# engyasin/EKF-MonoSLAM_for_3D-reconstruction

Measured on AMD Instinct MI355X. Metric: EKF updates/sec at N features (state dim 14+6N), higher is better.
Workload: dtype f32 (state, covariance, every accumulation and every other contraction in fp32; the products of the covariance downdate as 3 x bf16 splits of the fp32 operands, six bf16 products per fp32 product: the dropped terms are <= 2^-24 |a||b| in the worst case (2^-28 on average) -- the size of the fp32 prod; 1 GPU; N=1000 inverse-depth features, n=6014, M=N measured per frame, fp32, 1xMI355X (BASELINE configs[2]); features=1000, state_dim=6014, measured_per_frame=1000, camera=conf_kinect.cfg/scale2, frames_per_map=3000, maps=1

## Files before the change

### ekf-monoslam_for_3d-reconstruction_amd/csrc/ekf_capi.hip

```cpp
#include <hip/hip_runtime.h>

#include <algorithm>
#include <array>
#include <climits>
#include <cmath>
#include <cstdint>
#include <cstdio>
#include <cstdlib>
#include <cstring>
#include <map>
#include <mutex>
#include <string>
#include <type_traits>
#include <vector>

#include "../../include/ekf_monoslam.h"
#include "ekf_buffers.hpp"
#include "ekf_feature_table.hpp"
#include "ekf_dense.hpp"
#include "ekf_image.hpp"
#include "ekf_features.hpp"
#include "ekf_syrk6.hpp"
#include "ekf_chain.hpp"
#include "ekf_small.hpp"
// ... 41 lines not shown
  KID_SEED_MASK,
  KID_SEED_RESPONSE,
  KID_SEED_CANDIDATES,
  KID_SEED_SELECT,
  KID_FRAME_UPLOAD,
  KID_FRAME_INGEST,
  KID_FRAME_RECTIFY,
  KID_COUNT
};

static const char* kKernelNames[KID_COUNT] = {
    "predict_camera",  "propagate_strips", "propagate_streaming", "measure",
    "innovation",      "sigma_ht",         "innovation_cov",      "chol_diag",
    "chol_panel",      "chol_trailing",    "state_update",        "downdate_syrk",
    "solve_trmm",      "normalize_quat",  "add_feature",      "compact_transform",   "misc",
    "w_update", "allgather_h", "allgather_s", "allgather_v", "allgather_sigma",
    "seed_mask", "seed_response", "seed_candidates", "seed_select", "frame_upload", "frame_ingest", "frame_rectify"};

static const char* kLaunchNames[EKF_LAUNCH_KINDS] = {
    "downdate_bf16x6", "downdate_f32", "downdate_f32_fused_wu", "downdate_f32_half_tail", "downdate_f32_t64",
    "row_rider", "row_gemv", "row_tile_gemm", "w_update_gemm", "w_recompute",
    "chain_step_launches", "chain_persistent", "solve", "solve_two_groups", "update_oneblock", "update_allinone",
    "chain_trail_diag", "split_image", "state_update_tail", "update_onelaunch", "chain_dist_gather", "chain_step_fused",
    "downdate_mirror_bounds", "solve_poll_chain"};

static inline int round_up(int v, int a) { return (v + a - 1) / a * a; }

struct MaskedStreamPool {
  struct Entry { int device, num_cus, reserved; hipStream_t st; };
  std::mutex mu;
  std::vector<Entry> idle;
  bool hooked = false;
  static void at_exit();
  hipStream_t take(int device, int num_cus, int reserved) {
    std::lock_guard<std::mutex> lk(mu);
    for (size_t i = 0; i < idle.size(); ++i)
      if (idle[i].device == device && idle[i].num_cus == num_cus && idle[i].reserved == reserved) {
        hipStream_t st = idle[i].st;
        idle.erase(idle.begin() + i);
        return st;
      }
    return nullptr;
  }
  void give(int device, int num_cus, int reserved, hipStream_t st) {
    std::lock_guard<std::mutex> lk(mu);
    idle.push_back({device, num_cus, reserved, st});
    if (!hooked) { hooked = true; atexit(&MaskedStreamPool::at_exit); }
// ... 170 lines not shown
  DevBuf<unsigned char> d_raw;
  int raw_w = 0, raw_h = 0, raw_c = 0;
  bool have_raw = false;
  RectScratch rect;
  DevBuf<int4> d_ingest_tab;
  int ingest_tab_w = 0, ingest_tab_h = 0;
  DevBuf<unsigned char> d_patch[2], d_mpatch[2];
  int cur_patch = 0;
  DevBuf<T> d_hb, d_zm;
  DevBuf<unsigned char> d_found;
  DevBuf<float> d_score;
  DevBuf<int> d_keep;
  int opt_panel_direct = 1;
  int opt_chain_fused_diag = 1;
  int opt_small_onelaunch = 1;
  int opt_step_fused = 1;
  struct StepPlan { std::vector<int> off, cnt; } sfp;
  WorkList sf_lists{{0}, {}};
  DevBuf<unsigned long long> d_small_stamps;
  unsigned small_gate_total = 0;
  int opt_su_tail = 1;
  int opt_syrk_mirror_skip = 1;
  int opt_solve_poll_chain = 1;
  int opt_fuse_split = 1;
  int opt_chain_defer = 1;
  int td_min_blocks = 24;
  int td_max_blocks = 1 << 30;
  WorkList td_blocks;
  std::vector<int> td_off, td_cnt;
  int opt_syrk_stag_half = 0, opt_syrk_stag_mod4 = 2;
  int opt_solve_s2 = 1;
  bool want_solve_s2(int width, int npad_live) const {
    return kIsF32 && opt_mfma && opt_solve_s2 && (opt_solve_s2 > 1 || (width / 128) * (npad_live / 64) <= 2 * num_cus);
  }
  int opt_fused = 1;
  int opt_solve_one_per_cu = 1;
  int opt_wrecompute = 1;
  int opt_row_gemv = 1;
  int opt_fuse_wu = 1;
  int env_chunks[8] = {}, env_nchunks = 0;
  int opt_pipeline = -1;
  WorkList tilemap{{0, 0}, {}};
  int tri_count = 0, solve_off = 0;
  int w_zeroed_n = -1;
  DevBuf<int> d_counters;
  int num_cus = 256, reserved_cus = 32;
// ... 125 lines not shown
          stream_b = nullptr;
          reserved_cus = 0;
          HIPCHK(hipStreamCreateWithFlags(&stream_b, hipStreamNonBlocking));
        }
      }
      stream_b_reserved = reserved_cus;

      if (const char* e = getenv("EKF_FUSE_WU")) opt_fuse_wu = atoi(e);
      if (const char* e = getenv("EKF_ROW_GEMV")) opt_row_gemv = atoi(e) ? 1 : 0;
      if (const char* e = getenv("EKF_SOLVE_ONE_PER_CU")) opt_solve_one_per_cu = atoi(e) ? 1 : 0;
      if (const char* e = getenv("EKF_W_RECOMPUTE")) opt_wrecompute = atoi(e) ? 1 : 0;
      if (const char* e = getenv("EKF_SOLVE_S2")) opt_solve_s2 = atoi(e);
      if (const char* e = getenv("EKF_FUSED_LAUNCHES")) opt_fused = atoi(e) ? 1 : 0;
      if (const char* e = getenv("EKF_PANEL_DIRECT")) opt_panel_direct = atoi(e);
      if (const char* e = getenv("EKF_SYRK_STAGGER")) {
        opt_syrk_stag_half = atoi(e);
        if (const char* c = strchr(e, ',')) opt_syrk_stag_mod4 = atoi(c + 1);
      }
      if (const char* e = getenv("EKF_CHAIN_FUSED_DIAG")) opt_chain_fused_diag = atoi(e) ? 1 : 0;
      if (const char* e = getenv("EKF_FUSE_SPLIT")) opt_fuse_split = atoi(e) ? 1 : 0;
      if (const char* e = getenv("EKF_SU_TAIL")) opt_su_tail = atoi(e) ? 1 : 0;
      if (const char* e = getenv("EKF_SYRK_MIRROR_SKIP")) opt_syrk_mirror_skip = atoi(e) ? 1 : 0;
      if (const char* e = getenv("EKF_SOLVE_POLL_CHAIN")) opt_solve_poll_chain = std::max(0, std::min(2, atoi(e)));
      if (const char* e = getenv("EKF_SMALL_ONELAUNCH")) opt_small_onelaunch = atoi(e) ? 1 : 0;
      if (const char* e = getenv("EKF_STEP_FUSED")) opt_step_fused = atoi(e) ? 1 : 0;
      if (const char* e = getenv("EKF_SHARD_DIST_CHAIN")) opt_shard_dist_chain = atoi(e) ? 1 : 0;
      if (const char* e = getenv("EKF_SHARD_DIST_MIN_BLOCKS")) shard_dist_min_blocks = std::max(2, atoi(e));
      if (const char* e = getenv("EKF_SMALL_STAMPS")) {
        if (atoi(e)) { HIPCHK(d_small_stamps.reserve(16)); HIPCHK(hipMemset(d_small_stamps, 0, 16 * sizeof(unsigned long long))); }
      }
      if (const char* e = getenv("EKF_CHAIN_DEFER")) opt_chain_defer = atoi(e) ? 1 : 0;
      if (const char* e = getenv("EKF_TD_MIN_BLOCKS")) td_min_blocks = std::max(1, atoi(e));
      if (const char* e = getenv("EKF_TD_MAX_BLOCKS")) td_max_blocks = std::max(1, atoi(e));
      if (const char* e = getenv("EKF_SPLIT_TAIL")) opt_split_tail = atoi(e);
      if (const char* e = getenv("EKF_SPLIT_BF16")) opt_split_bf16 = atoi(e) ? 1 : 0;
      if (const char* e = getenv("EKF_CHUNKS")) {
        for (const char* q = e; *q && env_nchunks < 8;) {
          env_chunks[env_nchunks++] = atoi(q);
          while (*q && *q != ',') ++q;
          if (*q == ',') ++q;
        }
      }
    }
    std::vector<T> mu0(camera_dim, T(0));
    mu0[3] = T(0.0); mu0[4] = T(0.0); mu0[5] = T(-0.707106781); mu0[6] = T(0.707106781);
    if (camera_dim == 14) mu0[13] = T(1);
// ... 683 lines not shown
      int rc = zero_border(dst, n);
      if (rc) return rc;
      cur = dst;
    } else {
      Scope sc(this, KID_PROPAGATE_STRIPS);
      k_strip_congruence<T, 13><<<(2 * n + 255) / 256, 256, 0, stream>>>(S(), ld, n, 0, d_scr + SCR_FT, d_scr + SCR_Q);
    }
    if (opt_feature_noise > 0.0 && n > camera_dim)
      k_inflate_diagonal<T><<<(n - camera_dim + 255) / 256, 256, 0, stream>>>(S(), ld, camera_dim, n, T(opt_feature_noise));
    HIPCHK(hipGetLastError());
    return EKF_OK;
  }

  int predict(const void* tc, const void* rc_, int vcontrol) override {
    HIPCHK(hipSetDevice(device));
    if (sh_on) return shard_predict(tc, rc_, vcontrol);
    const MotionArgs a = motion_args(tc, rc_, vcontrol);
    if (opt_fused && !opt_streaming && !(opt_feature_noise > 0.0) && N > 0 && !prof.on(KID_PREDICT_CAMERA) &&
        !prof.on(KID_PROPAGATE_STRIPS) && !prof.on(KID_MEASURE)) {
      int rc = sync_layout();
      if (rc) return rc;
      const int nstrip = (2 * n + 255) / 256;
      k_predict_fused<T><<<nstrip + (N + 255) / 256, 256, 0, stream>>>(mu(), d_scr, a, S(), ld, n, nstrip, d_pos, d_coding, N,
                                                                      cam, d_h, d_Hc, d_Hf, d_flags, d_status + 8, d_status);
      HIPCHK(hipGetLastError());
      rc = launch_track_fold();
      if (rc) return rc;
      have_motion = true;
      have_update = false;
      have_meas = true;
      have_sd = false;
      return launch_blur();
    }
    int rcp = propagate(a, opt_streaming);
    if (rcp) return rcp;
    have_update = false;
    int rcm = launch_measure();
    if (rcm) return rcm;
    return launch_blur();
  }

  int measure() override {
    HIPCHK(hipSetDevice(device));
    return launch_measure();
  }

  bool have_motion = false;
  int motion_jacobian(void* Ft, void* Q) override {
    HIPCHK(hipSetDevice(device));
    if (!have_motion) FAIL(EKF_ERR_STATE, "no motion Jacobian: call ekf_predict first");
// ... 84 lines not shown
    int nb = 0, tile = 0, m = 0, m_pad = 0, npad_live = 0, nsteps = 0;
    int nchunks = 1, cend[8] = {};
    ChunkTab tab{};
    int strip_rows = 0;
    int ntr = 0, ntc = 0;
    bool oneblock = false, allinone = false, onelaunch = false;
    int small_rc = 0, small_nchunk = 0, small_nt64 = 0;
    bool recompute = false;
    int r0 = 0, r1 = 0, p0 = 0, prows = 0;
    Rows ranges[3] = {};
    bool sym_panel = false, shard_split = false;
    int c0(int g) const { return (g ? cend[g - 1] : 0) * nb; }
    int c1(int g) const { return cend[g] * nb; }
  };
  struct UpdateCtx {
    const T* z;
    const int* midx;
    int* counters;
    int counter_next = 0;
    bool step_fused = false;
    int diag_ahead = -1;
    struct { int step = -1, c0 = 0, c1 = 0; } pending;
    bool row_pending = false;
    bool queue_room(int ints = 8) const { return counter_next + ints <= kQueueCounters; }
    int* take_queue() {
      if (!queue_room()) return nullptr;
      counter_next += 8;
      return counters + counter_next - 8;
    }
  };

  template <int ROLE, bool BT, int TM = 128, int TN = 128>
  void gemm(const GemmCall& c) {
    GemmArgs g{};
    g.A = c.A; g.lda = c.lda; g.B = c.B; g.ldb = c.ldb; g.C = c.C; g.ldc = c.ldc;
    g.K = c.K; g.alpha = double(c.alpha); g.beta = double(c.beta);
    g.tri = c.tri; g.row_off = c.row_off; g.col_off = c.col_off; g.ktri = c.ktri; g.ktile_off = c.ktile_off;
    g.zrow = c.zrow; g.zcol_end = c.zcol_end;
    g.stagger = (ROLE == ROLE_DOWNDATE) ? 1 : 0;
    g.img = c.img; g.img_nkc = c.img_nkc; g.img_c0 = c.img_c0;
    g.chain_word = c.chain_word; g.chain_epoch = c.chain_epoch; g.status = d_status;
    hipStream_t st = c.st ? c.st : stream;
    const bool mf = kIsF32 && opt_mfma;
    dim3 grid(c.cols / (mf ? TN : 64), c.rows / (mf ? TM : 64));
    if (c.tile_list && c.counter) {
      g.tile_map = c.tile_list;
// ... 6 lines not shown
    }
    if constexpr (kIsF32) {
      if (opt_mfma) {
        if constexpr (ROLE == ROLE_SOLVE) {
          ++launch_cnt[c.two_groups ? EKF_LAUNCH_SOLVE_TWO_GROUPS : EKF_LAUNCH_SOLVE];
          if (c.two_groups) {
            k_gemm_mfma<ROLE, BT, TM, TN, true><<<grid, 512, 0, st>>>(g);
            return;
          }
        }
        k_gemm_mfma<ROLE, BT, TM, TN><<<grid, 256, 0, st>>>(g);
        return;
      }
    }
    if constexpr (!kIsF32) {
      if (opt_mfma) {
        k_gemm_mfma_f64<ROLE, BT><<<grid, 256, 0, st>>>(g);
        return;
      }
    }
    k_gemm_valu<T, ROLE, BT><<<grid, 256, 0, st>>>(g);
  }

  void launch_panel(T* P, const T* Dj, int vrows, hipStream_t st) {
    const int nb = NB();
    if constexpr (kIsF32) {
      if (opt_mfma && nb == 128 && opt_panel_direct) {
        k_panel_direct<<<(vrows + 63) / 64, 256, 0, st>>>(P, ldy, Dj, vrows);
        return;
      }
    }
    if constexpr (!kIsF32) {
      if (opt_mfma && nb == 64 && opt_panel_direct) {
        k_panel_direct_f64<<<(vrows + 63) / 64, 256, 0, st>>>(P, ldy, Dj, vrows);
        return;
      }
    }
    GemmCall c;
    c.A = P; c.lda = ldy; c.B = Dj; c.ldb = nb; c.C = P; c.ldc = ldy;
    c.rows = vrows; c.cols = nb; c.K = nb; c.st = st;
    gemm<ROLE_PANEL, false, 64, 128>(c);
  }

  int ensure_tilemap(int nt, int ntr, int ntc) {
    const std::vector<int> key = {nt, ntc};
    if (tilemap.current(key)) return EKF_OK;
    std::vector<int> tm;
    const int SB = 8;
    const int ns = (nt + SB - 1) / SB;
    for (int si = 0; si < ns; ++si)
      for (int sj = 0; sj <= si; ++sj)
// ... 279 lines not shown
      if (ux.diag_ahead != step) {
        Scope sc(this, KID_CHOL_DIAG, sc_);
        ++launch_cnt[EKF_LAUNCH_CHAIN_STEP];
        if (nb == 128) {
          if constexpr (kIsF32)
            k_chol_diag_packed<><<<1, 1024, 0, sc_>>>(Ajj, ldy, Dj, d_status, std::max(1, std::min(8, (m - j + 15) / 16)));
        } else {
          if constexpr (!kIsF32) {
            if (opt_mfma)
              k_chol_diag_packed_f64<<<1, 512, 0, sc_>>>(Ajj, ldy, Dj, d_status, std::max(1, std::min(4, (m - j + 15) / 16)));
            else
              k_chol_diag<T, 64><<<1, 512, diag_lds(64), sc_>>>(Ajj, ldy, Dj, d_status);
          } else {
            k_chol_diag<T, 64><<<1, 512, diag_lds(64), sc_>>>(Ajj, ldy, Dj, d_status);
          }
        }
      }
      const int r0 = j + nb;
      const int vrows = m_pad - c0;
      if (!skip_panel) {
        Scope sc(this, KID_CHOL_PANEL, sc_);
        T* P = Y + (size_t)r0 * ldy + j;
        ++launch_cnt[EKF_LAUNCH_CHAIN_STEP];
        launch_panel(P, Dj, vrows, sc_);
      }
      if (defer_last && step == step1 - 1 && r0 < m_pad) {
        ux.pending.step = step; ux.pending.c0 = c0; ux.pending.c1 = c1;
      } else {
        chain_trailing(ux, step, c0, c1, m, m_pad, sc_, !skip_panel);
      }
    }
  }
  int check_list(const int* idx, int M, bool ascending) {
    for (int k = 0; k < M; ++k) {
      if (idx[k] < 0 || idx[k] >= N) FAIL(EKF_ERR_ARG, "feature index out of range");
      if (ascending && k > 0 && idx[k - 1] >= idx[k]) FAIL(EKF_ERR_ARG, "measured indices must be strictly ascending");
    }
    return EKF_OK;
  }

  void launch_row_update(int c0, int c1, int m_pad, hipStream_t ss, bool gemv) {
    const size_t yrow = (size_t)round_up(n, NB()) * ldy;
    Scope sc(this, KID_WUPDATE, ss);
    ++launch_cnt[gemv ? EKF_LAUNCH_ROW_GEMV : EKF_LAUNCH_ROW_TILE_GEMM];
    if constexpr (kIsF32) {
      if (gemv) {
        k_innov_row_update<<<(m_pad - c1 + 63) / 64, 64, 0, ss>>>(d_V + yrow + c0, d_Y + (size_t)c1 * ldy + c0, ldy,
// ... 24 lines not shown
      Syrk6Args a{d_Vimg, ldy / 16, c0 / 16, width / 16, S(), ld, tiles, ntiles, head, cam_rows, r0, r1};
      a.stag_half = opt_syrk_stag_half; a.stag_mod4 = opt_syrk_stag_mod4;
      if (su_tail) {
        a.su_mu = mu(); a.su_V = d_V; a.su_ldy = ldy; a.su_n = n; a.su_y = d_V + (size_t)npad_live * ldy; a.su_mpad = m_pad;
        a.su_qn = d_scr + SCR_QN; a.su_counter = head + 1;
        ++launch_cnt[EKF_LAUNCH_STATE_UPDATE_TAIL];
      }
      if (rider) {
        a.ry = d_V + (size_t)npad_live * ldy + c0; a.rL = d_Y + (size_t)c1 * ldy + c0; a.rldl = ldy;
        a.rnu = d_W + (size_t)npad_live * ldy + c1; a.rcols = m_pad - c1; a.rK = width; a.nrider = (m_pad - c1 + 255) / 256;
        ++launch_cnt[EKF_LAUNCH_ROW_RIDER];
      }
      if (mirror_rows) {
        a.mirror_rows = mirror_rows;
        ++launch_cnt[EKF_LAUNCH_DOWNDATE_MIRROR_BOUNDS];
      }
      ++launch_cnt[EKF_LAUNCH_DOWNDATE_BF16X6];
      const int wgs = 2 * (ss == stream_b ? num_cus - reserved_cus : num_cus);
      k_syrk_bf16x6<0><<<a.nrider + std::min(ntiles, wgs), 256, 0, ss>>>(a);
    }
    return EKF_OK;
  }

  void launch_w_recompute(int c1, int c2, int m_pad, const int* list, int M, int plane, hipStream_t ss, int rows0,
                          int row0 = 0, int row1 = 0) {
    if constexpr (kIsF32) {
      Scope sc(this, KID_SIGMA_HT, ss);
      ++launch_cnt[EKF_LAUNCH_W_RECOMPUTE];
      const int s0 = c1 / 2, s1 = c2 / 2;
      const int range[2][2] = {{0, rows0}, {row0, row1}};
      for (const auto& r : range) {
        if (r[1] <= r[0]) continue;
        constexpr int RB = 8;
        dim3 grid((s1 - s0 + 127) / 128, (r[1] - r[0] + RB - 1) / RB);
        k_sigma_ht_fast<RB><<<grid, 256, 0, ss>>>(S(), ld, r[1], d_Hc, d_Hf, d_pos, d_coding, list, M, plane, d_W, ldy, m_pad, N,
                                                   s0, s1, nullptr, nullptr, nullptr, nullptr, nullptr, nullptr, nullptr, r[0]);
      }
    }
  }

  void launch_state_update(int m_pad, hipStream_t st) {
    Scope sc(this, KID_STATE_UPDATE, st);
    k_state_update<T><<<(n + 7) / 8, 512, 0, st>>>(mu(), d_V, ldy, n, d_V + (size_t)round_up(n, NB()) * ldy, m_pad, d_scr + SCR_QN);
  }

  int finish_update(const UpdatePlan& p, bool state_update, bool normalize) {
    last_nchunks = p.nchunks;
    last_recompute = p.recompute;
    for (int g = 0; g < p.nchunks; ++g) last_cend[g] = p.cend[g];
    if (state_update) launch_state_update(p.m_pad, stream);
    if (normalize) {
      Scope sc(this, KID_NORMALIZE);
      k_strip_congruence<T, 4><<<(2 * n + 255) / 256, 256, 0, stream>>>(S(), ld, n, 3, d_scr + SCR_QN,
                                                                       static_cast<const T*>(nullptr));
    }
    HIPCHK(hipGetLastError());
    last_m = p.m; last_m_pad = p.m_pad; last_n = n;
    have_update = true;
    have_meas = false;
// ... 54 lines not shown
        if (rc) return rc;
        ux.step_fused = true;
      }
    }
    return EKF_OK;
  }

  bool chunk_overlaps(const UpdatePlan& p, int g) const { return stream_b != nullptr && g + 1 < p.nchunks; }
  int chunk_slots(const UpdatePlan& p, int g) const { return 2 * (chunk_overlaps(p, g) ? num_cus - reserved_cus : num_cus); }
  bool chunk_splits(const UpdatePlan& p, const UpdateCtx& ux) const {
    return kIsF32 && opt_split_bf16 && opt_mfma && p.tile == 128 && tri_count >= num_cus && ux.queue_room();
  }
  bool chunk_fuses(const UpdatePlan& p, int g, const UpdateCtx& ux) const {
    return kIsF32 && opt_fuse_wu && (opt_fuse_wu > 1 || p.recompute || g + 2 < p.nchunks) && opt_mfma && chunk_overlaps(p, g) &&
           p.c1(g) < p.m_pad && !opt_split_bf16 && p.tile == 128 && tri_count >= num_cus && ux.queue_room();
  }
  bool chunk_row_rider(const UpdatePlan& p, int g, const UpdateCtx& ux) const {
    return chunk_splits(p, ux) && p.recompute && opt_row_gemv && p.c1(g) < p.m_pad && !chunk_fuses(p, g, ux);
  }
  bool chunk_su_tail(const UpdatePlan& p, int g, const UpdateCtx& ux) const {
    return kIsF32 && opt_su_tail && !chunk_overlaps(p, g) && p.nchunks > 1 && chunk_splits(p, ux);
  }
  bool solve_polls_chain(const UpdatePlan& p, int g) const {
    return kIsF32 && opt_mfma && opt_solve_poll_chain && (p.nsteps <= 16 || opt_solve_poll_chain > 1) && g > 0 &&
           chunk_overlaps(p, g) && stream_b_masked && reserved_cus > 0 && !p.oneblock;
  }
  enum SolveShape { SOLVE_64X64, SOLVE_128_ONE_PER_CU, SOLVE_64X128, SOLVE_128 };
  SolveShape solve_shape(const UpdatePlan& p, int g) const {
    const bool mf = kIsF32 && opt_mfma;
    const int tiles = (p.c1(g) - p.c0(g)) / p.tile * p.ntr, slots = chunk_slots(p, g);
    if (mf && 4 * tiles < slots) return SOLVE_64X64;
    if (mf && !chunk_overlaps(p, g) && opt_solve_one_per_cu && tiles < slots && tiles > num_cus) return SOLVE_128_ONE_PER_CU;
    if (mf && tiles < slots) return SOLVE_64X128;
    return SOLVE_128;
  }

  int launch_update_small(const UpdatePlan& p, const UpdateCtx& ux) {
    if constexpr (kIsF32) {
      if (w_zeroed_n != n) {
        HIPCHK(hipMemsetAsync(d_W + (size_t)n * ldy, 0, (size_t)(p.npad_live - n + p.nb) * ldy * sizeof(T), stream));
        w_zeroed_n = n;
      }
      SmallUpdateArgs a{};
      a.S = S(); a.ld = ld; a.n = n; a.npad = p.npad_live;
      a.Hc = d_Hc; a.Hf = d_Hf; a.pos = d_pos; a.coding = d_coding; a.midx = ux.midx;
      a.M = p.M; a.plane = p.plane; a.nfeat = N;
      a.z = ux.z; a.h = d_h; a.mu = mu();
      a.r_pix = T(sigma_pixel_2); a.r_plane = T(0.00001);
// ... 14 lines not shown
    const int c0 = p.c0(gi), width = p.c1(gi) - c0, ntr = p.ntr, ntc = p.ntc;
    T* Zs = d_Y + (size_t)p.m_pad * ldy;
    if (p.oneblock) {
      if constexpr (kIsF32) {
        ++launch_cnt[p.allinone ? EKF_LAUNCH_UPDATE_ALLINONE : EKF_LAUNCH_UPDATE_ONEBLOCK];
        if (p.allinone)
          k_update_oneblock_small<<<p.small_nt64 + 1, 512, 0, ss>>>(d_W, ldy, d_Dinv, d_V, ldy, p.npad_live, mu(), n, d_scr + SCR_QOLD,
                                                                   d_scr + SCR_QN, Zs, ldy, S(), ld, p.small_nt64);
        else
          k_solve_state_oneblock<<<p.npad_live / 64 + 1, 256, 0, ss>>>(d_W, ldy, d_Dinv, d_V, ldy, p.npad_live, mu(), n,
                                                                      d_scr + SCR_QN, Zs, ldy);
      }
      return EKF_OK;
    }
    Scope sc(this, KID_SOLVE, ss);
    const int wt = width / p.tile;
    GemmCall c;
    c.A = d_W + c0; c.lda = ldy; c.B = Zs + c0; c.ldb = ldy; c.C = d_V + c0; c.ldc = ldy;
    c.rows = p.npad_live + p.nb; c.cols = width; c.K = width; c.ktri = KTRI_UPPER;
    c.two_groups = want_solve_s2(width, p.npad_live);
    c.st = ss;
    if (ss == stream_b && solve_polls_chain(p, gi)) {
      c.chain_word = reinterpret_cast<const unsigned*>(d_counters + kChainEpochWord); c.chain_epoch = (unsigned)gi + 1;
      ++launch_cnt[EKF_LAUNCH_SOLVE_POLL_CHAIN];
    }
    switch (solve_shape(p, gi)) {
      case SOLVE_64X64:
        c.tile_list = tilemap.d + solve6464_off + 2 * (2 * ntc - 2 * wt) * 2 * ntr; c.ntiles = 2 * wt * 2 * ntr;
        c.counter = ux.take_queue();
        gemm<ROLE_SOLVE, true, 64, 64>(c);
        break;
      case SOLVE_128_ONE_PER_CU:
        c.tile_list = tilemap.d + solve_off + 2 * (ntc - wt) * ntr; c.ntiles = wt * ntr;
        c.counter = ux.take_queue();
        c.one_per_cu = true;
        gemm<ROLE_SOLVE, true>(c);
        break;
      case SOLVE_64X128:
        if (kIsF32 && opt_fuse_split && opt_split_bf16 && p.tile == 128 && tri_count >= num_cus && ux.queue_room(16)) {
          HIPCHK(ensure_vimg());
          c.img = d_Vimg; c.img_nkc = ldy / 16; c.img_c0 = c0;
          *vimg_done = true;
        }
        c.tile_list = tilemap.d + solve64_off + 2 * (ntc - wt) * 2 * ntr; c.ntiles = wt * 2 * ntr;
        c.counter = ux.take_queue();
        gemm<ROLE_SOLVE, true, 64, 128>(c);
        break;
// ... 104 lines not shown
    UpdateCtx ux{d_z, d_midx, d_counters};
    if (M > 0) {
      if (on_device) {
        ux.z = static_cast<const T*>(z);
        ux.midx = idx;
      } else {
        int rcs = stage_inputs(z, idx, M);
        if (rcs) return rcs;
        sh_list.clear();
      }
    }
    const UpdatePlan p = plan_update(M, plane);
    int rc = p.onelaunch ? launch_update_small(p, ux)
                         : build_innovation(ux.z, ux.midx, M, plane, true, nullptr, nullptr, &p.tab, p.strip_rows);
    if (rc) return rc;
    rc = ensure_tilemap(p.npad_live / p.tile, p.ntr, p.ntc);
    if (rc) return rc;
    rc = prepare_chain(p, ux, false);
    if (rc) return rc;
    const int nchunks = p.nchunks, m_pad = p.m_pad;
    bool b_inflight = false;
    for (int gi = 0; gi < (p.onelaunch ? 0 : nchunks); ++gi) {
      const int c0 = p.c0(gi), c1 = p.c1(gi);
      chain_steps(ux, gi ? p.cend[gi - 1] : 0, p.cend[gi], c0, c1, p.m, m_pad, stream, p.oneblock,
                  opt_chain_defer && gi + 1 < nchunks);
      const bool overlap = chunk_overlaps(p, gi);
      hipStream_t ss = overlap ? stream_b : stream;
      if (!overlap && b_inflight) {
        if (p.recompute) {
          HIPCHK(hipEventRecord(ev_b, stream_b));
          HIPCHK(hipStreamWaitEvent(stream, ev_b, 0));
          b_inflight = false;
        } else {
          HIPCHK(hipStreamWaitEvent(stream, ev_wu, 0));
        }
      }
      if (overlap) {
        b_inflight = true;
        if (solve_polls_chain(p, gi)) {
          if constexpr (kIsF32)
            k_publish_epoch<<<1, 64, 0, stream>>>(reinterpret_cast<unsigned*>(d_counters + kChainEpochWord), (unsigned)gi + 1);
        } else {
          HIPCHK(hipEventRecord(ev_chain[gi], stream));
          HIPCHK(hipStreamWaitEvent(stream_b, ev_chain[gi], 0));
        }
      }
      bool vimg_done = false;
      rc = solve_chunk(p, gi, ux, ss, &vimg_done);
      if (rc) return rc;
      const bool fuse = chunk_fuses(p, gi, ux);
      wupdate_chunk(p, gi, ux, ss);
      if (overlap && c1 < m_pad && !fuse && !p.recompute) HIPCHK(hipEventRecord(ev_wu, stream_b));
      if (!overlap && b_inflight) {
        HIPCHK(hipEventRecord(ev_b, stream_b));
        HIPCHK(hipStreamWaitEvent(stream, ev_b, 0));
        b_inflight = false;
      }
      if (!overlap && nchunks > 1 && !chunk_su_tail(p, gi, ux)) {
        HIPCHK(hipEventRecord(ev_chain[gi], stream));
        HIPCHK(hipStreamWaitEvent(stream_b, ev_chain[gi], 0));
        launch_state_update(m_pad, stream_b);
        b_inflight = true;
      }
      rc = downdate_chunk(p, gi, ux, ss, vimg_done);
// ... 3775 lines not shown
```

### ekf-monoslam_for_3d-reconstruction_amd/csrc/ekf_dense.hpp

```cpp
#pragma once
#include <type_traits>
#include "ekf_math.hpp"

namespace ekf {

typedef float f32x4 __attribute__((ext_vector_type(4)));
constexpr int kQueueCounters = 256;
constexpr int kChainEpochWord = kQueueCounters;
constexpr int kResetInts = kQueueCounters + 32;

__device__ __forceinline__ int clamp_feature(int fi, int nfeat) { return min(max(fi, 0), nfeat - 1); }
__device__ __forceinline__ void check_measured_entry(const int* __restrict__ midx, int k, int nfeat,
                                                     int* __restrict__ status) {
  const int fi = midx[k];
  if (status && (fi < 0 || fi >= nfeat || (k > 0 && midx[k - 1] >= fi))) status[1] = 1;
}

struct ChunkTab {
  int n;
  int end[8];
};

constexpr int kMirrorEmpty = 8;
constexpr int kMirrorRowsInts = 2 * (kMirrorEmpty + 1);
__device__ __forceinline__ void mirror_rows_slab(const ChunkTab& tab, const int* __restrict__ midx, int M, int nfeat,
                                                 const int* __restrict__ pos, const int* __restrict__ coding,
                                                 int* __restrict__ mrows) {
  __shared__ int s_lo[8], s_hi[8];
  const int tid = threadIdx.x;
  if (tid < 8) { s_lo[tid] = 0x7fffffff; s_hi[tid] = 0; }
  __syncthreads();
  for (int k = tid; k < M; k += blockDim.x) {
// ... 1360 lines not shown
      f4 acc = {0.f, 0.f, 0.f, 0.f};
      const float* bl = sl + (16 * ct + lr) * PITCH + 4 * lq;
#pragma unroll
      for (int u = 0; u < 8; ++u) {
        if (u <= ct) {
          const f4 fb = *reinterpret_cast<const f4*>(bl + 16 * u);
#pragma unroll
          for (int e = 0; e < 4; ++e) acc = __builtin_amdgcn_mfma_f32_16x16x4f32(fa[u][e], fb[e], acc, 0, 0, 0);
        }
      }
#pragma unroll
      for (int e = 0; e < 4; ++e) P[(size_t)(row0 + 4 * lq + e) * ldp + 16 * ct + lr] = acc[e];
    }
  };
  if (live) column_tiles(0);
#pragma unroll
  for (int p = 0; p < 8; ++p) {
    const int q = tid + 256 * p;
    *reinterpret_cast<f4*>(sl + (64 + (q >> 5)) * PITCH + 4 * (q & 31)) = v1[p];
  }
  __syncthreads();
  if (live) column_tiles(4);
}
__global__ void __launch_bounds__(256, 2) k_panel_direct(float* __restrict__ P, int ldp, const float* __restrict__ Dinv, int rows) {
  __shared__ float sl[128 * 132];
  panel_direct_body(P, ldp, Dinv, rows, blockIdx.x, sl);
}
__global__ void __launch_bounds__(256, 2) k_panel_direct_blocks(float* __restrict__ Pcol, int ldp, const float* __restrict__ Dinv,
                                                               const int* __restrict__ blocks) {
  __shared__ float sl[128 * 132];
  const int blk = blocks[blockIdx.x >> 1];
  panel_direct_body(Pcol + (size_t)blk * 128 * ldp, ldp, Dinv, 128, blockIdx.x & 1, sl);
}

namespace oneblock {
constexpr int NB = 128, PITCH = 132;
typedef float f4 __attribute__((ext_vector_type(4)));

__device__ __forceinline__ void stage(const float* __restrict__ Dinv, const float* __restrict__ nu, float* sl, float* snu, int tid) {
  f4 v[16];
#pragma unroll
  for (int p = 0; p < 16; ++p) {
    const int q = tid + 256 * p;
    v[p] = *reinterpret_cast<const f4*>(Dinv + (size_t)(q >> 5) * NB + 4 * (q & 31));
  }
#pragma unroll
  for (int p = 0; p < 16; ++p) {
    const int q = tid + 256 * p;
    *reinterpret_cast<f4*>(sl + (q >> 5) * PITCH + 4 * (q & 31)) = v[p];
// ... 595 lines not shown
```

### ekf-monoslam_for_3d-reconstruction_amd/csrc/ekf_kernels.hpp

```cpp
#pragma once
#include "ekf_math.hpp"

namespace ekf {

enum : int {
  SCR_FT = 0,
  SCR_Q = 169,
  SCR_QN = 338,
  SCR_G = 354,
  SCR_C = 396,
  SCR_QOLD = 432,
  SCR_SIZE = 512
};

struct MotionArgs {
  double dT;
  double t_ctl[3];
  double r_ctl[3];
  double vdiag[6];
};

template <typename T>
__device__ __forceinline__ void camera_step(const T* sx, const MotionArgs& a, T* sF, T* xn) {
  const T dTt = T(a.dT);
// ... 314 lines not shown
  drot_dq_times(qc, d, Jq);
  for (int a = 0; a < 2; ++a) {
    for (int c = 0; c < 3; ++c) hc[a * 7 + c] = scale_r * JR[a * 3 + c];
    for (int c = 0; c < 4; ++c) {
      T acc = Jp[a * 3 + 0] * Jq[0 * 4 + c] + Jp[a * 3 + 1] * Jq[1 * 4 + c] + Jp[a * 3 + 2] * Jq[2 * 4 + c];
      hc[a * 7 + 3 + c] = (c == 0) ? acc : -acc;
    }
    for (int c = 0; c < fs; ++c)
      hf[a * 6 + c] = JR[a * 3 + 0] * Jf[0 * 6 + c] + JR[a * 3 + 1] * Jf[1 * 6 + c] + JR[a * 3 + 2] * Jf[2 * 6 + c];
  }
  h_out[2 * i] = hd[0];
  h_out[2 * i + 1] = hd[1];
  for (int k = 0; k < 14; ++k) Hc[(size_t)i * 14 + k] = hc[k];
  for (int k = 0; k < 12; ++k) Hf[(size_t)i * 12 + k] = hf[k];
  flags[i] = fl;
}

template <typename T>
__global__ void __launch_bounds__(256) k_predict_fused(T* __restrict__ mu, T* __restrict__ scr, MotionArgs a,
                                                       T* __restrict__ S, int ld, int n, int nstrip,
                                                       const int* __restrict__ pos, const int* __restrict__ coding, int N,
                                                       CamParams cam, T* __restrict__ h_out, T* __restrict__ Hc,
                                                       T* __restrict__ Hf, unsigned char* __restrict__ flags,
                                                       int* __restrict__ gate, int* __restrict__ status) {
  __shared__ T sF[169];
  __shared__ T sQ[169];
  __shared__ T sC[169];
  __shared__ T sA[169];
  __shared__ T sx[13];
  __shared__ T sxn[13];
  const int tid = threadIdx.x, bid = blockIdx.x;
  const bool strip = bid < nstrip;
  if (tid < 13) sx[tid] = mu[tid];
  for (int i = tid; i < 169; i += 256) sF[i] = (i / 13 == i % 13) ? T(1) : T(0);
  __syncthreads();
  if (tid == 0) {
    if (bid != 0) __hip_atomic_fetch_add(gate, 1, __ATOMIC_RELAXED, __HIP_MEMORY_SCOPE_AGENT);
    camera_step(sx, a, strip ? sF : static_cast<T*>(nullptr), sxn);
  }
  __syncthreads();
  if (!strip) {
    const int i = (bid - nstrip) * 256 + tid;
    if (i < N) measure_feature<T>(i, mu, pos, coding, cam, h_out, Hc, Hf, flags, sxn);
    return;
  }
  if (bid == 0) {
    for (int e = tid; e < 169; e += 256) {
      const T qv = process_noise_entry(sF, a, e);
      sQ[e] = qv;
      scr[SCR_FT + e] = sF[e];
      scr[SCR_Q + e] = qv;
    }
    __syncthreads();
  }
  strip_congruence_body<T, 13>(S, ld, n, 0, sF, sQ, sC, sA, bid, tid, 256);
  if (bid == 0 && tid == 0) {
    bool ok = false;
    for (int spin = 0; spin < (1 << 20) && !ok; ++spin) {
      ok = __hip_atomic_load(gate, __ATOMIC_RELAXED, __HIP_MEMORY_SCOPE_AGENT) >= (int)gridDim.x - 1;
      if (!ok) __builtin_amdgcn_s_sleep(8);
    }
    if (!ok) status[3] = 1;
    for (int k = 0; k < 13; ++k) mu[k] = sxn[k];
    __hip_atomic_store(gate, 0, __ATOMIC_RELAXED, __HIP_MEMORY_SCOPE_AGENT);
  }
}
// ... 497 lines not shown
```

### include/ekf_monoslam.h

```cpp
#ifndef EKF_MONOSLAM_H_
#define EKF_MONOSLAM_H_

#include <stddef.h>

#ifdef __cplusplus
extern "C" {
#endif

#define EKF_ABI_VERSION 6

typedef struct ekf_filter ekf_filter;

enum ekf_dtype { EKF_F32 = 0, EKF_F64 = 1 };

enum ekf_status {
  EKF_OK = 0,
  EKF_ERR_ARG = 1,
  EKF_ERR_CAPACITY = 2,
  EKF_ERR_DEVICE = 3,
  EKF_ERR_STATE = 4,
  EKF_ERR_NUMERIC = 5,
  EKF_ERR_UNSUPPORTED = 6
};

// ... 118 lines not shown
  EKF_LAUNCH_DOWNDATE_F32,
  EKF_LAUNCH_DOWNDATE_F32_FUSED_WU,
  EKF_LAUNCH_DOWNDATE_F32_HALF_TAIL,
  EKF_LAUNCH_DOWNDATE_F32_T64,
  EKF_LAUNCH_ROW_RIDER,
  EKF_LAUNCH_ROW_GEMV,
  EKF_LAUNCH_ROW_TILE_GEMM,
  EKF_LAUNCH_W_UPDATE_GEMM,
  EKF_LAUNCH_W_RECOMPUTE,
  EKF_LAUNCH_CHAIN_STEP,
  EKF_LAUNCH_CHAIN_PERSISTENT,
  EKF_LAUNCH_SOLVE,
  EKF_LAUNCH_SOLVE_TWO_GROUPS,
  EKF_LAUNCH_UPDATE_ONEBLOCK,
  EKF_LAUNCH_UPDATE_ALLINONE,
  EKF_LAUNCH_CHAIN_TRAIL_DIAG,
  EKF_LAUNCH_SPLIT_IMAGE,
  EKF_LAUNCH_STATE_UPDATE_TAIL,
  EKF_LAUNCH_UPDATE_ONELAUNCH,
  EKF_LAUNCH_CHAIN_DIST_GATHER,
  EKF_LAUNCH_CHAIN_STEP_FUSED,
  EKF_LAUNCH_DOWNDATE_MIRROR_BOUNDS,
  EKF_LAUNCH_SOLVE_POLL_CHAIN,
  EKF_LAUNCH_KINDS
};
int ekf_launch_kinds(void);
const char* ekf_launch_kind_name(int kind);
int ekf_launch_count(ekf_filter* f, int kind, long long* launches);

typedef int (*ekf_allgather_fn)(void* ctx, const void* d_send, void* d_recv, size_t bytes_per_rank, void* hip_stream);

typedef struct ekf_shard_info {
  int rank, world, N, state_dim;
  int f_begin, f_end;
  int row_begin, row_end;
  int max_rows_any_rank;
  int rebalances;
} ekf_shard_info;

int ekf_shard_configure(ekf_filter* f, int rank, int world, ekf_allgather_fn allgather, void* ctx);
int ekf_shard_get_info(ekf_filter* f, ekf_shard_info* out);
int ekf_shard_update(ekf_filter* f, const void* d_z, const int* indices, int M, int plane_constraint);
int ekf_shard_rebalance(ekf_filter* f);

void* ekf_device_mu(ekf_filter* f);
void* ekf_device_sigma(ekf_filter* f, int* ld);
// ... 168 lines not shown
```

Measured before the change: 1157 updates/s.

## Fuse track fold into predict kernel and add optional chain publish/solve tweaks

The predict kernel now folds the per-feature tracking flags inline, so the separate track-fold launch is skipped by default. It also adds three options that are off by default: the epoch can be published from inside the last panel kernel through an arrival counter; the first solve chunk can poll the chain early behind an event; and sigma_ht row blocks are picked by a wave-quantization rule. The default path saves one small kernel launch per predict, at the cost of extra read-modify-write traffic on the track array inside the measurement blocks.

Result: no change. 1164 updates/s, median of 6 (+0.6%).

```diff
diff --git a/ekf-monoslam_for_3d-reconstruction_amd/csrc/ekf_capi.hip b/ekf-monoslam_for_3d-reconstruction_amd/csrc/ekf_capi.hip
--- a/ekf-monoslam_for_3d-reconstruction_amd/csrc/ekf_capi.hip
+++ b/ekf-monoslam_for_3d-reconstruction_amd/csrc/ekf_capi.hip
@@ -87,7 +87,8 @@
     "row_rider", "row_gemv", "row_tile_gemm", "w_update_gemm", "w_recompute",
     "chain_step_launches", "chain_persistent", "solve", "solve_two_groups", "update_oneblock", "update_allinone",
     "chain_trail_diag", "split_image", "state_update_tail", "update_onelaunch", "chain_dist_gather", "chain_step_fused",
-    "downdate_mirror_bounds", "solve_poll_chain"};
+    "downdate_mirror_bounds", "solve_poll_chain", "publish_epoch", "publish_in_panel", "solve0_early",
+    "w_recompute_wave_rule"};
 
 static inline int round_up(int v, int a) { return (v + a - 1) / a * a; }
 
@@ -304,6 +305,10 @@
   int opt_su_tail = 1;
   int opt_syrk_mirror_skip = 1;
   int opt_solve_poll_chain = 1;
+  int opt_track_fold_fused = 1;
+  int opt_publish_in_panel = 0;
+  int opt_solve0_early = 0;
+  int opt_wrec_full_waves = 0;
   int opt_fuse_split = 1;
   int opt_chain_defer = 1;
   int td_min_blocks = 24;
@@ -475,6 +480,10 @@
       if (const char* e = getenv("EKF_SU_TAIL")) opt_su_tail = atoi(e) ? 1 : 0;
       if (const char* e = getenv("EKF_SYRK_MIRROR_SKIP")) opt_syrk_mirror_skip = atoi(e) ? 1 : 0;
       if (const char* e = getenv("EKF_SOLVE_POLL_CHAIN")) opt_solve_poll_chain = std::max(0, std::min(2, atoi(e)));
+      if (const char* e = getenv("EKF_TRACK_FOLD_FUSED")) opt_track_fold_fused = atoi(e) ? 1 : 0;
+      if (const char* e = getenv("EKF_PUBLISH_IN_PANEL")) opt_publish_in_panel = atoi(e) ? 1 : 0;
+      if (const char* e = getenv("EKF_SOLVE0_EARLY")) opt_solve0_early = atoi(e) ? 1 : 0;
+      if (const char* e = getenv("EKF_WREC_FULL_WAVES")) opt_wrec_full_waves = std::max(0, atoi(e));
       if (const char* e = getenv("EKF_SMALL_ONELAUNCH")) opt_small_onelaunch = atoi(e) ? 1 : 0;
       if (const char* e = getenv("EKF_STEP_FUSED")) opt_step_fused = atoi(e) ? 1 : 0;
       if (const char* e = getenv("EKF_SHARD_DIST_CHAIN")) opt_shard_dist_chain = atoi(e) ? 1 : 0;
@@ -1204,10 +1213,15 @@
       if (rc) return rc;
       const int nstrip = (2 * n + 255) / 256;
       k_predict_fused<T><<<nstrip + (N + 255) / 256, 256, 0, stream>>>(mu(), d_scr, a, S(), ld, n, nstrip, d_pos, d_coding, N,
-                                                                      cam, d_h, d_Hc, d_Hf, d_flags, d_status + 8, d_status);
+                                                                      cam, d_h, d_Hc, d_Hf, d_flags, d_status + 8, d_status,
+                                                                      opt_track_fold_fused ? static_cast<unsigned char*>(d_trk) : nullptr);
       HIPCHK(hipGetLastError());
-      rc = launch_track_fold();
-      if (rc) return rc;
+      if (opt_track_fold_fused) {
+        trk_dirty = true;
+      } else {
+        rc = launch_track_fold();
+        if (rc) return rc;
+      }
       have_motion = true;
       have_update = false;
       have_meas = true;
@@ -1338,6 +1352,9 @@
     int diag_ahead = -1;
     struct { int step = -1, c0 = 0, c1 = 0; } pending;
     bool row_pending = false;
+    unsigned publish_epoch = 0;
+    hipEvent_t early_event = nullptr;
+    hipError_t early_rc = hipSuccess;
     bool queue_room(int ints = 8) const { return counter_next + ints <= kQueueCounters; }
     int* take_queue() {
       if (!queue_room()) return nullptr;
@@ -1390,11 +1407,17 @@
     k_gemm_valu<T, ROLE, BT><<<grid, 256, 0, st>>>(g);
   }
 
-  void launch_panel(T* P, const T* Dj, int vrows, hipStream_t st) {
+  void launch_panel(T* P, const T* Dj, int vrows, hipStream_t st, unsigned publish = 0) {
     const int nb = NB();
     if constexpr (kIsF32) {
       if (opt_mfma && nb == 128 && opt_panel_direct) {
-        k_panel_direct<<<(vrows + 63) / 64, 256, 0, st>>>(P, ldy, Dj, vrows);
+        if (publish) {
+          ++launch_cnt[EKF_LAUNCH_PUBLISH_IN_PANEL];
+          k_panel_direct<<<(vrows + 63) / 64, 256, 0, st>>>(P, ldy, Dj, vrows, reinterpret_cast<unsigned*>(d_counters + kChainEpochWord),
+                                                            d_counters + kChainArriveWord, publish);
+        } else {
+          k_panel_direct<<<(vrows + 63) / 64, 256, 0, st>>>(P, ldy, Dj, vrows);
+        }
         return;
       }
     }
@@ -1720,7 +1743,9 @@
         Scope sc(this, KID_CHOL_PANEL, sc_);
         T* P = Y + (size_t)r0 * ldy + j;
         ++launch_cnt[EKF_LAUNCH_CHAIN_STEP];
-        launch_panel(P, Dj, vrows, sc_);
+        const bool chunk_last = defer_last && step == step1 - 1;
+        if (chunk_last && ux.early_event) ux.early_rc = hipEventRecord(ux.early_event, sc_);
+        launch_panel(P, Dj, vrows, sc_, chunk_last ? ux.publish_epoch : 0u);
       }
       if (defer_last && step == step1 - 1 && r0 < m_pad) {
         ux.pending.step = step; ux.pending.c0 = c0; ux.pending.c1 = c1;
@@ -1791,6 +1816,18 @@
     return EKF_OK;
   }
 
+  int wrec_row_block(int gx, int rows, hipStream_t ss) const {
+    if (opt_wrec_full_waves == 0 || opt_wrec_full_waves == 8) return 8;
+    if (opt_wrec_full_waves == 16) return 16;
+    const int cus = (ss == stream_b && stream_b_masked) ? num_cus - reserved_cus : num_cus;
+    double idle[2];
+    for (int k = 0; k < 2; ++k) {
+      const int rb = 8 << k, wgs = gx * ((rows + rb - 1) / rb), resident = (k ? 3 : 6) * cus;
+      const int waves = (wgs + resident - 1) / resident;
+      idle[k] = waves <= 1 ? 0.0 : double(waves) - double(wgs) / resident;
+    }
+    return idle[1] < idle[0] ? 16 : 8;
+  }
   void launch_w_recompute(int c1, int c2, int m_pad, const int* list, int M, int plane, hipStream_t ss, int rows0,
                           int row0 = 0, int row1 = 0) {
     if constexpr (kIsF32) {
@@ -1800,10 +1837,17 @@
       const int range[2][2] = {{0, rows0}, {row0, row1}};
       for (const auto& r : range) {
         if (r[1] <= r[0]) continue;
-        constexpr int RB = 8;
-        dim3 grid((s1 - s0 + 127) / 128, (r[1] - r[0] + RB - 1) / RB);
-        k_sigma_ht_fast<RB><<<grid, 256, 0, ss>>>(S(), ld, r[1], d_Hc, d_Hf, d_pos, d_coding, list, M, plane, d_W, ldy, m_pad, N,
+        const int gx = (s1 - s0 + 127) / 128, rows = r[1] - r[0];
+        if (opt_wrec_full_waves) ++launch_cnt[EKF_LAUNCH_W_RECOMPUTE_WAVE_RULE];
+        if (wrec_row_block(gx, rows, ss) == 16) {
+          dim3 grid(gx, (rows + 15) / 16);
+          k_sigma_ht_fast<16><<<grid, 256, 0, ss>>>(S(), ld, r[1], d_Hc, d_Hf, d_pos, d_coding, list, M, plane, d_W, ldy, m_pad, N,
+                                                    s0, s1, nullptr, nullptr, nullptr, nullptr, nullptr, nullptr, nullptr, r[0]);
+        } else {
+          dim3 grid(gx, (rows + 7) / 8);
+          k_sigma_ht_fast<8><<<grid, 256, 0, ss>>>(S(), ld, r[1], d_Hc, d_Hf, d_pos, d_coding, list, M, plane, d_W, ldy, m_pad, N,
                                                    s0, s1, nullptr, nullptr, nullptr, nullptr, nullptr, nullptr, nullptr, r[0]);
+        }
       }
     }
   }
@@ -1904,8 +1948,12 @@
     return kIsF32 && opt_su_tail && !chunk_overlaps(p, g) && p.nchunks > 1 && chunk_splits(p, ux);
   }
   bool solve_polls_chain(const UpdatePlan& p, int g) const {
-    return kIsF32 && opt_mfma && opt_solve_poll_chain && (p.nsteps <= 16 || opt_solve_poll_chain > 1) && g > 0 &&
+    return kIsF32 && opt_mfma && opt_solve_poll_chain && (p.nsteps <= 16 || opt_solve_poll_chain > 1) && (g > 0 || solve0_early(p)) &&
            chunk_overlaps(p, g) && stream_b_masked && reserved_cus > 0 && !p.oneblock;
+  }
+  bool solve0_early(const UpdatePlan& p) const { return opt_solve0_early && opt_chain_defer && opt_panel_direct && p.nb == 128; }
+  bool chunk_publishes_in_panel(const UpdatePlan& p, int g) const {
+    return opt_publish_in_panel && opt_chain_defer && opt_panel_direct && p.nb == 128 && solve_polls_chain(p, g);
   }
   enum SolveShape { SOLVE_64X64, SOLVE_128_ONE_PER_CU, SOLVE_64X128, SOLVE_128 };
   SolveShape solve_shape(const UpdatePlan& p, int g) const {
@@ -1966,7 +2014,7 @@
     c.st = ss;
     if (ss == stream_b && solve_polls_chain(p, gi)) {
       c.chain_word = reinterpret_cast<const unsigned*>(d_counters + kChainEpochWord); c.chain_epoch = (unsigned)gi + 1;
-      ++launch_cnt[EKF_LAUNCH_SOLVE_POLL_CHAIN];
+      ++launch_cnt[gi ? EKF_LAUNCH_SOLVE_POLL_CHAIN : EKF_LAUNCH_SOLVE0_EARLY];
     }
     switch (solve_shape(p, gi)) {
       case SOLVE_64X64:
@@ -2117,6 +2165,9 @@
     bool b_inflight = false;
     for (int gi = 0; gi < (p.onelaunch ? 0 : nchunks); ++gi) {
       const int c0 = p.c0(gi), c1 = p.c1(gi);
+      const bool polls = solve_polls_chain(p, gi), in_panel = chunk_publishes_in_panel(p, gi);
+      ux.publish_epoch = in_panel ? (unsigned)gi + 1 : 0u;
+      ux.early_event = (polls && gi == 0) ? ev_chain[0] : nullptr;
       chain_steps(ux, gi ? p.cend[gi - 1] : 0, p.cend[gi], c0, c1, p.m, m_pad, stream, p.oneblock,
                   opt_chain_defer && gi + 1 < nchunks);
       const bool overlap = chunk_overlaps(p, gi);
@@ -2132,9 +2183,17 @@
       }
       if (overlap) {
         b_inflight = true;
-        if (solve_polls_chain(p, gi)) {
-          if constexpr (kIsF32)
-            k_publish_epoch<<<1, 64, 0, stream>>>(reinterpret_cast<unsigned*>(d_counters + kChainEpochWord), (unsigned)gi + 1);
+        if (polls) {
+          if (gi == 0) {
+            HIPCHK(ux.early_rc);
+            HIPCHK(hipStreamWaitEvent(stream_b, ev_chain[0], 0));
+          }
+          if constexpr (kIsF32) {
+            if (!in_panel) {
+              ++launch_cnt[EKF_LAUNCH_PUBLISH_EPOCH];
+              k_publish_epoch<<<1, 64, 0, stream>>>(reinterpret_cast<unsigned*>(d_counters + kChainEpochWord), (unsigned)gi + 1);
+            }
+          }
         } else {
           HIPCHK(hipEventRecord(ev_chain[gi], stream));
           HIPCHK(hipStreamWaitEvent(stream_b, ev_chain[gi], 0));
diff --git a/ekf-monoslam_for_3d-reconstruction_amd/csrc/ekf_dense.hpp b/ekf-monoslam_for_3d-reconstruction_amd/csrc/ekf_dense.hpp
--- a/ekf-monoslam_for_3d-reconstruction_amd/csrc/ekf_dense.hpp
+++ b/ekf-monoslam_for_3d-reconstruction_amd/csrc/ekf_dense.hpp
@@ -7,7 +7,8 @@
 typedef float f32x4 __attribute__((ext_vector_type(4)));
 constexpr int kQueueCounters = 256;
 constexpr int kChainEpochWord = kQueueCounters;
-constexpr int kResetInts = kQueueCounters + 32;
+constexpr int kChainArriveWord = kQueueCounters + 32;
+constexpr int kResetInts = kQueueCounters + 64;
 
 __device__ __forceinline__ int clamp_feature(int fi, int nfeat) { return min(max(fi, 0), nfeat - 1); }
 __device__ __forceinline__ void check_measured_entry(const int* __restrict__ midx, int k, int nfeat,
@@ -1414,9 +1415,22 @@
   __syncthreads();
   if (live) column_tiles(4);
 }
-__global__ void __launch_bounds__(256, 2) k_panel_direct(float* __restrict__ P, int ldp, const float* __restrict__ Dinv, int rows) {
+__global__ void __launch_bounds__(256, 2) k_panel_direct(float* __restrict__ P, int ldp, const float* __restrict__ Dinv, int rows,
+                                                         unsigned* __restrict__ epoch_word = nullptr, int* __restrict__ arrive = nullptr,
+                                                         unsigned epoch = 0) {
   __shared__ float sl[128 * 132];
   panel_direct_body(P, ldp, Dinv, rows, blockIdx.x, sl);
+  if (epoch_word != nullptr) {
+    __syncthreads();
+    if (threadIdx.x == 0) {
+      const int before = __hip_atomic_fetch_add(arrive, 1, __ATOMIC_RELEASE, __HIP_MEMORY_SCOPE_AGENT);
+      if (before == (int)gridDim.x - 1) {
+        __builtin_amdgcn_fence(__ATOMIC_ACQ_REL, "agent");
+        __hip_atomic_store(arrive, 0, __ATOMIC_RELAXED, __HIP_MEMORY_SCOPE_AGENT);
+        __hip_atomic_store(epoch_word, epoch, __ATOMIC_RELAXED, __HIP_MEMORY_SCOPE_AGENT);
+      }
+    }
+  }
 }
 __global__ void __launch_bounds__(256, 2) k_panel_direct_blocks(float* __restrict__ Pcol, int ldp, const float* __restrict__ Dinv,
                                                                const int* __restrict__ blocks) {
diff --git a/ekf-monoslam_for_3d-reconstruction_amd/csrc/ekf_kernels.hpp b/ekf-monoslam_for_3d-reconstruction_amd/csrc/ekf_kernels.hpp
--- a/ekf-monoslam_for_3d-reconstruction_amd/csrc/ekf_kernels.hpp
+++ b/ekf-monoslam_for_3d-reconstruction_amd/csrc/ekf_kernels.hpp
@@ -360,7 +360,8 @@
                                                        const int* __restrict__ pos, const int* __restrict__ coding, int N,
                                                        CamParams cam, T* __restrict__ h_out, T* __restrict__ Hc,
                                                        T* __restrict__ Hf, unsigned char* __restrict__ flags,
-                                                       int* __restrict__ gate, int* __restrict__ status) {
+                                                       int* __restrict__ gate, int* __restrict__ status,
+                                                       unsigned char* __restrict__ trk) {
   __shared__ T sF[169];
   __shared__ T sQ[169];
   __shared__ T sC[169];
@@ -379,7 +380,13 @@
   __syncthreads();
   if (!strip) {
     const int i = (bid - nstrip) * 256 + tid;
-    if (i < N) measure_feature<T>(i, mu, pos, coding, cam, h_out, Hc, Hf, flags, sxn);
+    if (i < N) {
+      measure_feature<T>(i, mu, pos, coding, cam, h_out, Hc, Hf, flags, sxn);
+      if (trk) {
+        const unsigned char fl = flags[i];
+        trk[i] = (unsigned char)((fl & 1) | (trk[i] & 2) | (fl & 2));
+      }
+    }
     return;
   }
   if (bid == 0) {
diff --git a/include/ekf_monoslam.h b/include/ekf_monoslam.h
--- a/include/ekf_monoslam.h
+++ b/include/ekf_monoslam.h
@@ -164,6 +164,10 @@
   EKF_LAUNCH_CHAIN_STEP_FUSED,
   EKF_LAUNCH_DOWNDATE_MIRROR_BOUNDS,
   EKF_LAUNCH_SOLVE_POLL_CHAIN,
+  EKF_LAUNCH_PUBLISH_EPOCH,
+  EKF_LAUNCH_PUBLISH_IN_PANEL,
+  EKF_LAUNCH_SOLVE0_EARLY,
+  EKF_LAUNCH_W_RECOMPUTE_WAVE_RULE,
   EKF_LAUNCH_KINDS
 };
 int ekf_launch_kinds(void);
```
